# CVMI-Lab/DODA

Hardware: AMD Instinct MI355X
Metric: active-voxels/sec fwd+bwd SparseConv U-Net, ScanNet 2cm (higher is better)
Workload: dtype bf16; 1 GPU; cfgs/scannet SparseConv U-Net training step (voxel pooling + fwd + CE + bwd + SGD), 2 cm voxels, 4 scenes/GPU x ~150000 active voxels, random-init weights; global_batch=4, voxels_per_gpu=601279, points_per_gpu=781042, parallelism=dp1, n_classes=20, grad_sync=deferred multi-layer wgrad + bucketed all-reduce, collectives=none (single process), prefetch_gate=off, grad_exchange=no process group

## Files before the change

doda_amd/_lib.py:

```python
import ctypes as C
import os

_HERE = os.path.dirname(os.path.abspath(__file__))
LIB_PATH = os.path.join(_HERE, "libdoda_hip.so")

c_i32, c_i64, c_f32, c_sz, c_vp = C.c_int32, C.c_int64, C.c_float, C.c_size_t, C.c_void_p

_SIGNATURES = {
    "doda_abi_version": (c_i32, []),
    "doda_strerror": (C.c_char_p, [c_i32]),
    "doda_voxelize_idx_h": (c_i32, [c_vp, c_i32, c_i32, c_i32, c_i32, c_vp, C.POINTER(c_vp),
                                    C.POINTER(c_i32), C.POINTER(c_i32)]),
    "doda_voxelize_idx_fill_h": (c_i32, [c_vp, c_vp, c_vp, c_vp]),
    "doda_voxelize_idx_free_h": (None, [c_vp]),
    "doda_voxelize_idx_workspace_bytes": (c_sz, [c_i32]),
    "doda_voxelize_idx_assign": (c_i32, [c_vp, c_i32, c_i32, c_i32, c_vp, c_vp, c_vp, c_sz, c_vp]),
    "doda_voxelize_idx_fill": (c_i32, [c_vp, c_i32, c_i32, c_i32, c_i32, c_i32, c_vp, c_vp, c_vp,
                                       c_sz, c_vp]),
    "doda_voxelize_fp": (c_i32, [c_vp, c_vp, c_vp, c_i32, c_i32, c_i32, c_i32, c_vp]),
    "doda_voxelize_bp": (c_i32, [c_vp, c_vp, c_vp, c_i32, c_i32, c_i32, c_i32, c_vp]),
    "doda_voxelize_fp_rows": (c_i32, [c_vp, c_i32, c_vp, c_i32, c_vp, c_i32, c_i32, c_i32, c_vp, c_i32, c_i32, c_vp]),
    "doda_point_recover_fp": (c_i32, [c_vp, c_vp, c_vp, c_i32, c_i32, c_i32, c_vp]),
    "doda_point_recover_bp": (c_i32, [c_vp, c_vp, c_vp, c_i32, c_i32, c_i32, c_vp]),
    "doda_rulebook_workspace_bytes": (c_sz, [c_i32]),
# ... 121 lines not shown
    "doda_lovasz_bwd": (c_i32, [c_vp, c_i32, c_i32, c_i32, c_vp, c_vp, c_i32, c_vp, c_vp, c_vp, c_vp, c_vp, c_vp, c_vp, c_i32, c_vp]),
}
LOSS_SYMBOLS = tuple(LOSS_SIGNATURES)
LOSS_ABI_VERSION = 1
LOVASZ_MAX_CLASSES, LOVASZ_MAX_POINTS_PER_VOXEL = 32, 65535


class EvalScene(C.Structure):
    _fields_ = [("n_end", c_i32), ("m_end", c_i32), ("cell_base", c_i32), ("dims", c_i32 * 3), ("origin", c_f32 * 3),
                ("side", c_f32), ("inv_side", c_f32)]


EVAL_SIGNATURES = {
    "doda_eval_abi_version": (c_i32, []),
    "doda_eval_nn": (c_i32, [c_vp, c_vp, c_i64, c_vp, C.POINTER(EvalScene), c_i32, c_vp, c_vp, c_i64, c_vp, c_vp, c_vp]),
    "doda_eval_score_blocks": (c_i32, [c_i64]),
    "doda_eval_score": (c_i32, [c_vp, c_i32, c_i32, c_i32, c_vp, c_vp, c_i32, c_vp, c_i64, c_vp, c_vp, c_i64, c_i64, c_vp, c_vp, c_vp,
                                c_vp, c_i32, c_vp]),
}
EVAL_SYMBOLS = tuple(EVAL_SIGNATURES)
EVAL_ABI_VERSION = 1
EVAL_MAX_SCENES, EVAL_MAX_CELLS, EVAL_MAX_CLASSES = 32, 1 << 21, 32

c_u64p = C.POINTER(C.c_uint64)
SUBSAMPLE_SIGNATURES = {
    "doda_subsample_abi_version": (c_i32, []),
    "doda_subsample_workspace_bytes": (c_sz, [c_i64p, c_i32]),
    "doda_subsample_draw": (c_i32, [c_vp, c_vp, c_vp, c_vp, c_i64p, c_i32, c_i32p, c_u64p, C.c_uint32, c_vp, c_vp, c_vp, c_vp, c_vp,
                                    c_vp, c_sz, c_vp]),
}
SUBSAMPLE_SYMBOLS = tuple(SUBSAMPLE_SIGNATURES)
SUBSAMPLE_ABI_VERSION = 1
SUBSAMPLE_MAX_SEGMENTS, SUBSAMPLE_CHUNK = 64, 1024
OPT_TILE_KERNEL, OPT_WLDS_KERNEL, OPT_WDMA_KERNEL, OPT_TILE_PIPELINE, OPT_TILE_DUAL, OPT_CONV_UP = 1, 2, 3, 4, 5, 6
OPT_PRE_FWD_ROWS, OPT_PRE_BWD_ROWS = 7, 8
ABI_VERSION = 12

_ABIS = ((_SIGNATURES, "doda_abi_version", ABI_VERSION, "ABI"),
         (SELFTRAIN_SIGNATURES, "doda_st_abi_version", ST_ABI_VERSION, "self-training ABI"),
         (MIX_SIGNATURES, "doda_mix_abi_version", MIX_ABI_VERSION, "cuboid-mixing ABI"),
         (AUG_SIGNATURES, "doda_aug_abi_version", AUG_ABI_VERSION, "augmentation ABI"),
         (LOSS_SIGNATURES, "doda_loss_abi_version", LOSS_ABI_VERSION, "loss ABI"),
         (EVAL_SIGNATURES, "doda_eval_abi_version", EVAL_ABI_VERSION, "evaluation ABI"),
         (SUBSAMPLE_SIGNATURES, "doda_subsample_abi_version", SUBSAMPLE_ABI_VERSION, "subsample ABI"))

_lib = None


class DodaNativeError(RuntimeError):
    pass


def lib():
    global _lib
    if _lib is None:
        if not os.path.exists(LIB_PATH):
            raise DodaNativeError(
                "libdoda_hip.so is not built (%s). Run `python -m doda_amd.build` "
                "(hipcc, gfx950). doda_amd has no CPU fallback for its native ops." % LIB_PATH)
        handle = C.CDLL(LIB_PATH)
        for table, version_fn, version, what in _ABIS:
            for name, (res, args) in table.items():
                try:
                    fn = getattr(handle, name)
                except AttributeError as e:
                    raise DodaNativeError("libdoda_hip.so lacks symbol %s (stale build?)" % name) from e
                fn.restype = res
                fn.argtypes = args
            if getattr(handle, version_fn)() != version:
                raise DodaNativeError("libdoda_hip.so %s version mismatch" % what)
        _lib = handle
    return _lib


def check(status, what):
    if status != 0:
        msg = lib().doda_strerror(status).decode()
# ... 2 lines not shown
```

doda_amd/csrc/head.hip:

```cpp
#include "common.hpp"
#include "spconv_common.hpp"
#include "head_common.hpp"
#include "../../include/doda_selftrain.h"

namespace {

template <int ESZ, int C, int NK>
__global__ __launch_bounds__(HD_BLOCK, 4) void head_ce_fwd(const void *__restrict__ feats, int m, const float *__restrict__ weight,
                                                        const float *__restrict__ bias, int n_cls, const int32_t *__restrict__ v2p,
                                                        int v2p_ld, const long long *__restrict__ labels, long long ignore_index,
                                                        float *__restrict__ partial, int32_t *__restrict__ pred) {
    __shared__ float w[HD_MAX_K][HD_MAX_C], b[HD_MAX_K];
    __shared__ float red[2][HD_BLOCK / 64];
    hd_stage_weights<ESZ>(weight, bias, n_cls, C, w, b);
    float loss = 0.f, cnt = 0.f;
#pragma unroll 1
    for (long long v = (long long)blockIdx.x * HD_BLOCK + threadIdx.x; v < m; v += (long long)gridDim.x * HD_BLOCK) {
        asm volatile("" ::: "memory");
        float f[C], z[NK], mx;
        int arg;
        hd_load_row<ESZ, C>(feats, v, f);
        const int32_t *row = v2p + v * v2p_ld;
        const int np = row[0];
        hd_logits<C, NK>(w, b, n_cls, f, z, mx, arg);
        if (pred) pred[v] = arg;
        float s = 0.f;
#pragma unroll
        for (int k = 0; k < NK; ++k) s += __expf(z[k] - mx);
        const float lse = mx + __logf(s);
#pragma unroll 1
        for (int i = 0; i < np; ++i) {
            const long long lab = labels[row[1 + i]];
            if (lab != ignore_index && lab >= 0 && lab < n_cls) {
                float zy = 0.f;
#pragma unroll
                for (int k = 0; k < NK; ++k) zy = (int)lab == k ? z[k] : zy;
// ... 146 lines not shown
            }
            if (n_cls & 1) sdz[wid][n_cls - 1][lane] = r[n_cls - 1];
        } else {
#pragma unroll
            for (int c = 0; c < 16; ++c) sf[wid][c][lane] = 0;
            for (int k = 0; k < n_cls; ++k) sdz[wid][k][lane] = 0;
        }
        asm volatile("s_waitcnt lgkmcnt(0)" ::: "memory");
#pragma unroll
        for (int st = 0; st < 2; ++st) {
            const u32x4 bv = *reinterpret_cast<const u32x4 *>(&sf[wid][i][32 * st + 8 * g]);
#pragma unroll
            for (int t = 0; t < 2; ++t) {
                const u32x4 av = *reinterpret_cast<const u32x4 *>(&sdz[wid][16 * t + i][32 * st + 8 * g]);
                mma_bf16_k32(acc[t], av, bv);
            }
        }
        asm volatile("s_waitcnt lgkmcnt(0)" ::: "memory");
    }
    if (wid > 0) { red[wid - 1][0][lane] = acc[0]; red[wid - 1][1][lane] = acc[1]; }
    doda_sync();
    if (wid == 0) {
#pragma unroll
        for (int t = 0; t < 2; ++t) {
            f32x4 a = acc[t];
#pragma unroll
            for (int q = 0; q < 3; ++q) a += red[q][t][lane];
#pragma unroll
            for (int r = 0; r < 4; ++r) partial[(size_t)blockIdx.x * 512 + (size_t)(16 * t + 4 * g + r) * 16 + i] = a[r];
        }
    }
}

}

extern "C" int32_t doda_head_ce_blocks(int32_t m) { return hd_blocks(m > 0 ? m : 1); }

extern "C" int doda_head_ce_fwd(const void *feats, int32_t m, int32_t c, int32_t elem_bytes, const float *weight, const float *bias,
                                int32_t n_cls, const int32_t *v2p, int32_t v2p_ld, const int64_t *labels, int64_t ignore_index,
                                float *out, int32_t *pred, float *partial_ws, int32_t n_blocks, doda_stream_t stream) {
    if (!out) return DODA_ERR_INVALID;
    hipStream_t s = as_stream(stream);
    if (m == 0) { (void)hipMemsetAsync(out, 0, 8, s); return DODA_OK; }
    if (hd_args_bad(m, elem_bytes, v2p_ld, {feats, weight, v2p, labels, partial_ws}) || n_cls <= 0) return DODA_ERR_INVALID;
    if (c != 16 || n_cls > 32) return DODA_ERR_UNSUPPORTED;
    if (n_blocks != hd_blocks(m)) return DODA_ERR_WORKSPACE;
    HD_DISPATCH(head_ce_fwd, 16, n_blocks, feats, m, weight, bias, n_cls, v2p, v2p_ld, (const long long *)labels, (long long)ignore_index,
                partial_ws, pred);
    hipLaunchKernelGGL(head_ce_final, dim3(1), dim3(1024), 0, s, (const float *)partial_ws, n_blocks, out);
    return doda_check_launch();
}

extern "C" int doda_head_ce_bwd(const void *feats, int32_t m, int32_t c, int32_t elem_bytes, const float *weight, const float *bias,
                                int32_t n_cls, const int32_t *v2p, int32_t v2p_ld, const int64_t *labels, int64_t ignore_index,
                                const float *out, const float *grad, void *d_feats, void *dz, float *db_partial, int32_t n_blocks,
                                doda_stream_t stream) {
    if (m == 0) return DODA_OK;
    if (hd_args_bad(m, elem_bytes, v2p_ld, {feats, weight, v2p, labels, out, grad, d_feats, dz, db_partial}) || n_cls <= 0)
        return DODA_ERR_INVALID;
    if (c != 16 || n_cls > 32) return DODA_ERR_UNSUPPORTED;
    if (n_blocks != hd_blocks(m)) return DODA_ERR_WORKSPACE;
    hipStream_t s = as_stream(stream);
    HD_DISPATCH(head_ce_bwd, 16, n_blocks, feats, m, weight, bias, n_cls, v2p, v2p_ld, (const long long *)labels, (long long)ignore_index,
                out, grad, d_feats, dz, db_partial);
    return doda_check_launch();
}
// ... 29 lines not shown
```

doda_amd/csrc/spconv_gather.hip:

```cpp
#include <cstdio>
#include "common.hpp"
#include "tilebook.hpp"
#include "spconv_common.hpp"
#include "wgrad_backends.hpp"
#include <stdlib.h>

namespace {

struct F32 {
    typedef float elem;
    typedef f32x4 frag;
    static __device__ __forceinline__ frag zero() { return (frag){0.f, 0.f, 0.f, 0.f}; }
    static __device__ __forceinline__ elem from_float(float f) { return f; }
    static __device__ __forceinline__ float to_float(elem e) { return e; }
    static __device__ __forceinline__ void mma(f32x4 &acc, const frag &w, const frag &x) {
        mma_f32_k16<false>(acc, __builtin_bit_cast(u32x4, w), __builtin_bit_cast(u32x4, x));
    }
    static __device__ __forceinline__ void store4(elem *p, const f32x4 &v) {
        *reinterpret_cast<f32x4 *>(p) = v;
    }
};

struct BF16 {
    typedef unsigned short elem;
    typedef s16x4 frag;
    static __device__ __forceinline__ frag zero() { return (frag){0, 0, 0, 0}; }
    static __device__ __forceinline__ elem from_float(float f) { return f2bf(f); }
    static __device__ __forceinline__ float to_float(elem e) { return __uint_as_float((unsigned)e << 16); }
    static __device__ __forceinline__ void mma(f32x4 &acc, const frag &w, const frag &x) {
        acc = __builtin_amdgcn_mfma_f32_16x16x16bf16_1k(w, x, acc, 0, 0, 0);
    }
    static __device__ __forceinline__ void store4(elem *p, const f32x4 &v) {
        s16x4 o;
#pragma unroll
        for (int q = 0; q < 4; ++q) o[q] = (short)f2bf(v[q]);
        *reinterpret_cast<s16x4 *>(p) = o;
    }
// ... 92 lines not shown
            else f = d.w[((long long)((d.layout & 3) == 2 ? d.K - 1 - o : o) * d.nc + col) * d.kc + c];
        }
        v[q] = T::from_float(f);
    }
    reinterpret_cast<typename T::frag *>(d.out)[e] = v;
}

__global__ __launch_bounds__(256) void pack_weights_multi(const PackDesc *__restrict__ descs,
                                                          const int *__restrict__ blk_end, int n_desc) {
    int lo = 0, hi = n_desc - 1;
    while (lo < hi) {
        const int mid = (lo + hi) >> 1;
        if ((int)blockIdx.x < blk_end[mid]) hi = mid; else lo = mid + 1;
    }
    const PackDesc d = descs[lo];
    const int first = lo == 0 ? 0 : blk_end[lo - 1];
    const unsigned e = (unsigned)(blockIdx.x - first) * 256u + threadIdx.x;
    if (d.layout & 0x20) {
        if (e >= (unsigned)d.K * (unsigned)d.NB * 32u) return;
        const unsigned r = e >> 5, o = r / (unsigned)d.NB;
        reinterpret_cast<u32x4_t *>(d.out)[e] =
            pack_wide_frag(d.w, d.K, d.kc, d.nc, d.layout & 3, (int)o, 0, (int)(r - o * (unsigned)d.NB), (int)(e & 31));
        return;
    }
    const unsigned total = (unsigned)d.K * (unsigned)d.n_chunk * (unsigned)d.NB * 64u;
    if (e >= total) return;
    if (d.layout & 0x10) {
        const unsigned r = e >> 6, r1 = r / (unsigned)d.NB, nb = r - r1 * (unsigned)d.NB;
        const unsigned o = r1 / (unsigned)d.n_chunk, cc = r1 - o * (unsigned)d.n_chunk;
        reinterpret_cast<u32x4_t *>(d.out)[e] =
            pack_wide_frag(d.w, d.K, d.kc, d.nc, d.layout & 3, (int)o, (int)cc, (int)nb, (int)(e & 63));
    } else if (d.elem_bytes == 4) pack_one<F32>(d, e);
    else pack_one<BF16>(d, e);
}

constexpr int MAX_K = 27;

template <class T, int NBW, int S>
__global__ __launch_bounds__(256) void conv_gather(const typename T::elem *__restrict__ x, int kc,
                                                   const typename T::frag *__restrict__ wp, int nc,
                                                   int NB, const int32_t *__restrict__ tbl, int ld,
                                                   int K, int n_out,
                                                   typename T::elem *__restrict__ y, int vec_ok,
                                                   const typename T::elem *__restrict__ res) {
    typedef typename T::frag frag;
    typedef typename T::elem elem;
    constexpr int TM = 4 * 16 * S;
    __shared__ int32_t idx_tile[MAX_K * TM];

    const int lane = threadIdx.x & 63, wid = threadIdx.x >> 6;
    const int i = lane & 15, g = lane >> 4;
    const int n_nbg = (NB + NBW - 1) / NBW;
    const int item = xcd_work_item(blockIdx.x, gridDim.x);
    const long long r0 = (long long)(item / n_nbg) * TM;
    const int nb0 = (item % n_nbg) * NBW;

    for (int e = threadIdx.x; e < K * TM; e += 256) {
        const int o = e / TM, r = e - o * TM;
        idx_tile[e] = (r0 + r < n_out) ? tbl[(long long)o * ld + r0 + r] : -1;
    }
    doda_sync();

    const int wrow = wid * 16 * S;
    if (r0 + wrow >= n_out) return;

    unsigned int active = 0;
// ... 716 lines not shown
}

extern "C" size_t doda_spconv_pack_desc_bytes(void) { return sizeof(PackDesc); }

extern "C" int doda_spconv_pack_plan_h(void *descs_h, int32_t n_desc, int32_t *blk_end_h,
                                       int32_t *total_blocks) {
    if (!descs_h || !blk_end_h || !total_blocks || n_desc <= 0) return DODA_ERR_INVALID;
    PackDesc *d = (PackDesc *)descs_h;
    long long acc = 0;
    for (int k = 0; k < n_desc; ++k) {
        if (d[k].K <= 0 || d[k].K > MAX_K || d[k].kc <= 0 || d[k].nc <= 0 || (d[k].layout & ~3) ||
            (d[k].layout & 3) > 2 || (d[k].elem_bytes != 2 && d[k].elem_bytes != 4))
            return DODA_ERR_INVALID;
        const PackGeometry g = pack_geometry(d[k].K, d[k].kc, d[k].nc, d[k].elem_bytes);
        d[k].layout |= g.mode;
        d[k].n_chunk = g.n_chunk;
        d[k].NB = g.NB;
        acc += div_up(g.frags, 256);
        if (acc > 0x7fffffff) return DODA_ERR_UNSUPPORTED;
        blk_end_h[k] = (int32_t)acc;
    }
    *total_blocks = (int32_t)acc;
    return DODA_OK;
}

extern "C" int doda_spconv_pack_multi(const void *descs_dev, const int32_t *blk_end_dev,
                                      int32_t n_desc, int32_t total_blocks, doda_stream_t stream) {
    if (!descs_dev || !blk_end_dev || n_desc <= 0 || total_blocks <= 0) return DODA_ERR_INVALID;
    hipLaunchKernelGGL(pack_weights_multi, dim3(total_blocks), dim3(256), 0, as_stream(stream),
                       (const PackDesc *)descs_dev, blk_end_dev, n_desc);
    return doda_check_launch();
}

static bool *gather_switch(int32_t option) {
    switch (option) {
    case DODA_OPT_TILE_KERNEL: return &gather_switches().tile;
    case DODA_OPT_WLDS_KERNEL: return &gather_switches().wlds;
    case DODA_OPT_TILE_PIPELINE: return &gather_switches().tile_pipeline;
    case DODA_OPT_TILE_DUAL: return &gather_switches().tile_dual;
    case DODA_OPT_CONV_UP: return &gather_switches().conv_up;
    default: return nullptr;
    }
}
extern "C" int doda_set_option(int32_t option, int32_t value) {
    if (bool *sw = gather_switch(option)) { *sw = value != 0; return DODA_OK; }
    switch (option) {
    case DODA_OPT_WDMA_KERNEL: doda_wdma::set_enabled(value != 0); return DODA_OK;
    case DODA_OPT_PRE_FWD_ROWS: doda_layers::set_fwd_rows(value); return DODA_OK;
    case DODA_OPT_PRE_BWD_ROWS: doda_layers::set_bwd_rows(value); return DODA_OK;
    default: return DODA_ERR_INVALID;
    }
}
extern "C" int32_t doda_get_option(int32_t option) {
    if (const bool *sw = gather_switch(option)) return *sw ? 1 : 0;
    switch (option) {
    case DODA_OPT_WDMA_KERNEL: return doda_wdma::enabled() ? 1 : 0;
    case DODA_OPT_PRE_FWD_ROWS: return (int32_t)doda_layers::fwd_rows();
    case DODA_OPT_PRE_BWD_ROWS: return (int32_t)doda_layers::bwd_rows();
    default: return -1;
    }
}

extern "C" size_t doda_spconv_stats_capacity(int32_t n_out) { return n_out > 0 ? (size_t)div_up(n_out, 16) : 1; }

namespace doda_gather {
const GatherSwitches &switches() { return gather_switches(); }
// ... 60 lines not shown
```

doda_amd/csrc/spconv_wdma.hip:

```cpp
#include "tilebook.hpp"
#include "spconv_common.hpp"
#include "wgrad_common.hpp"
#include <stdlib.h>
#include <type_traits>
#include <string.h>

namespace {

constexpr int WD_WAVES = 16;
constexpr int WD_ROWS_BYTES = (TB_UMAX + 1) * 32;
constexpr int WD_LIDX_BYTES = TB_LIDX_BYTES;
constexpr int WD_DY_BYTES = TB_T * 32;
constexpr int WD_UNITS_BYTES = 2 * TB_K * 256 * 4;
constexpr int WD_BUF_BYTES = (WD_ROWS_BYTES + WD_LIDX_BYTES + WD_DY_BYTES) > WD_UNITS_BYTES ? (WD_ROWS_BYTES + WD_LIDX_BYTES + WD_DY_BYTES)
                                                                                           : WD_UNITS_BYTES;
static_assert(WD_LIDX_BYTES % 1024 == 0, "whole DMA pieces");
constexpr int WD_UNITS = 2 * TB_K;
constexpr int WD_MAX_UNITS = (WD_UNITS + WD_WAVES - 1) / WD_WAVES;
constexpr int WD_MAX_JOBS = 16;
static_assert(WD_BUF_BYTES % 16 == 0 && 2 * WD_BUF_BYTES + 64 <= 160 * 1024, "two tile buffers per CU");
static_assert(WD_UNITS * 256 * 4 <= WD_BUF_BYTES, "the final exchange re-uses ONE tile buffer (the other may be a DMA target)");

struct WdJob { const void *x, *dy; float *part; unsigned x_stride, dy_stride; int first_rank, pad; };
struct WdJobs { int n; WdJob j[WD_MAX_JOBS]; };
// ... 232 lines not shown
            const int o = e >> 8, c = e & 255;
            dst[e] = ex[(2 * o) * 256 + c] + ex[(2 * o + 1) * 256 + c];
        }
        asm volatile("s_waitcnt lgkmcnt(0)\n\ts_barrier" ::: "memory");
        if (tid < 2) reinterpret_cast<u32x4 *>(smem + bufsel * WD_BUF_BYTES)[tid] = (u32x4){0u, 0u, 0u, 0u};
        asm volatile("s_waitcnt lgkmcnt(0)\n\ts_barrier" ::: "memory");
    };

    bool nl_cur = __builtin_amdgcn_readfirstlane((int)la[0]) == -2;
    for (int item = 0; item < n_items; item += 2) {
        asm volatile("s_waitcnt vmcnt(0)" : "+v"(lb) : : "memory");
        asm volatile("s_waitcnt lgkmcnt(0)\n\ts_barrier" ::: "memory");
        {
            const bool nl_next = __builtin_amdgcn_readfirstlane((int)lb[0]) == -2;
            body(item, nl_cur, lb, la);
            nl_cur = nl_next;
        }
        if (item + 1 == n_items || (start + item + 1) % nt == 0) flush((start + item) / nt, item & 1, start + item);
        if (item + 1 >= n_items) break;
        asm volatile("s_waitcnt vmcnt(0)" : "+v"(la) : : "memory");
        asm volatile("s_waitcnt lgkmcnt(0)\n\ts_barrier" ::: "memory");
        {
            const bool nl_next = __builtin_amdgcn_readfirstlane((int)la[0]) == -2;
            body(item + 1, nl_cur, la, lb);
            nl_cur = nl_next;
        }
        if (item + 2 == n_items || (start + item + 2) % nt == 0) flush((start + item + 1) / nt, (item + 1) & 1, start + item + 1);
    }
    asm volatile("s_waitcnt vmcnt(0)" ::: "memory");
}

struct WdRJob { const float *part; float *dw; int accumulate, ldo, ldc, n_part; };
struct WdRJobs { WdRJob j[WD_MAX_JOBS]; };

__global__ __launch_bounds__(512) void wgrad_dma_reduce(const WdRJobs jobs) {
    __shared__ float red[16][32];
    const WdRJob d = jobs.j[blockIdx.y];
    const int n_part = d.n_part;
    const int jx = threadIdx.x & 31, p = threadIdx.x >> 5;
    const int e = blockIdx.x * 32 + jx;
    float a[8];
#pragma unroll
    for (int q = 0; q < 8; ++q) a[q] = 0.f;
    int b = p;
    for (; b + 7 * 16 < n_part; b += 8 * 16) {
#pragma unroll
        for (int q = 0; q < 8; ++q) a[q] += d.part[(size_t)(b + q * 16) * (TB_K * 256) + e];
    }
    for (int q = 0; b < n_part; b += 16, ++q) a[q & 7] += d.part[(size_t)b * (TB_K * 256) + e];
    red[p][jx] = ((a[0] + a[1]) + (a[2] + a[3])) + ((a[4] + a[5]) + (a[6] + a[7]));
    doda_sync();
    if (p == 0) {
        float v = 0.f;
#pragma unroll
        for (int q = 0; q < 16; ++q) v += red[q][jx];
        float *dst = d.dw + (size_t)(e >> 8) * d.ldo + (size_t)((e >> 4) & 15) * d.ldc + (e & 15);
        *dst = d.accumulate ? *dst + v : v;
    }
}

static_assert(WP_TILE_ROWS == TB_T && WP_TILE_K == TB_K, "wgrad_plan.hpp restates these constants");

struct Block { const void *x, *dy; float *dw; int x_stride, dy_stride, ldo, ldc, accumulate; };
struct WdArgs { WdJobs jobs; WdRJobs red; };

}

namespace doda_wdma {
// ... 38 lines not shown
            const int nj = l.n_blocks - first < WD_MAX_JOBS ? l.n_blocks - first : WD_MAX_JOBS;
            WdArgs a;
            ::memset(&a, 0, sizeof(a));
            a.jobs.n = nj;
            int first_rank[WD_MAX_JOBS], count[WD_MAX_JOBS];
            for (int k = 0; k < nj; ++k) { first_rank[k] = -1; count[k] = 0; }
            const long long N = (long long)nj * nt;
            if (N >= groups) {
                for (int r = 0; r < groups; ++r) {
                    const long long st = (long long)r * N / groups, en = (long long)(r + 1) * N / groups;
                    for (long long b = st / nt; b <= (en - 1) / nt; ++b) {
                        if (first_rank[b] < 0) first_rank[b] = r;
                        ++count[b];
                    }
                }
            } else {
                for (int k = 0; k < nj; ++k) { first_rank[k] = 0; count[k] = nt; }
            }
            for (int k = 0; k < nj; ++k) {
                const Block &b = blocks[first + k];
                float *pp = (float *)(part + used);
                used += (size_t)count[k] * TB_K * 256 * sizeof(float);
                a.jobs.j[k] = WdJob{b.x, b.dy, pp, (unsigned)b.x_stride, (unsigned)b.dy_stride, first_rank[k], 0};
                a.red.j[k] = WdRJob{pp, b.dw, b.accumulate, b.ldo, b.ldc, count[k]};
            }
            const unsigned char *bytes = (const unsigned char *)&a;
            p.args.insert(p.args.end(), bytes, bytes + sizeof(a));
        }
    }
}

int launch(const Plan &p, const doda_wgrad_job *jobs, hipStream_t s) {
    const WdArgs *a = (const WdArgs *)p.args.data();
    for (const Plan::Launch &l : p.launches) {
        const doda_wgrad_job &j0 = jobs[p.order[l.first_job]];
        const TileBookView tb = tilebook_view(const_cast<void *>(j0.tilebook), j0.n_rows);
        for (int first = 0; first < l.n_blocks; first += WD_MAX_JOBS, ++a) {
            doda_wgrad::trace("wgrad_dma16", wdma_groups(j0.n_rows), 1024, a->jobs.n);
            hipLaunchKernelGGL(wgrad_dma16, dim3(wdma_groups(j0.n_rows)), dim3(1024), 0, s, a->jobs, j0.tbl, j0.ld, j0.n_rows, tb);
            doda_wgrad::trace("wgrad_dma_reduce", TB_K * 256 / 32 * a->jobs.n, 512, a->jobs.n);
            hipLaunchKernelGGL(wgrad_dma_reduce, dim3(TB_K * 256 / 32, a->jobs.n), dim3(512), 0, s, a->red);
        }
    }
    return doda_check_launch();
}

}
```

doda_amd/model.py:

```python
import functools
from collections import OrderedDict
from types import SimpleNamespace

import torch
from torch import nn
from torch.autograd import Function

from torch.nn.modules import module as _torch_module

from . import ops as _ops
from . import pointgroup_ops, spconv
from .spconv import conv as _cv
from .spconv import functional as Fsp
from .spconv.modules import SparseModule


def default_cfg(n_classes=20, in_channel=3, mid_channel=16, block_reps=2, block_residual=True,
                use_xyz=False, voxel_mode=4):
    backbone = SimpleNamespace(in_channel=in_channel, mid_channel=mid_channel, block_reps=block_reps,
                               block_residual=block_residual, use_xyz=use_xyz)
    return SimpleNamespace(MODEL=SimpleNamespace(BACKBONE=backbone),
                           COMMON_CLASSES=SimpleNamespace(n_classes=n_classes),
                           DATA_CONFIG=SimpleNamespace(
                               DATA_PROCESSOR=SimpleNamespace(voxel_mode=voxel_mode),
# ... 472 lines not shown
            d_b = d_scores.sum(0)
        return d_feats, d_w, d_b, None, None


class _FusedCE(Function):
    @staticmethod
    def forward(ctx, scores, labels, ignore_index):
        scores = scores.contiguous()
        out, lse = _ops.cross_entropy_fwd(scores, labels, ignore_index)
        ctx.save_for_backward(scores, labels, lse, out)
        ctx.ignore_index = ignore_index
        return out[0]

    @staticmethod
    def backward(ctx, grad):
        scores, labels, lse, out = ctx.saved_tensors
        g = grad.reshape(1).to(torch.float32).contiguous()
        return _ops.cross_entropy_bwd(scores, labels, lse, out, g, ctx.ignore_index), None, None


class _VoxelHeadCE(Function):

    @staticmethod
    def forward(ctx, feats, weight, bias, v2p, labels, ignore_index):
        out, pred = _ops.head_ce_fwd(feats, weight, bias, v2p, labels, ignore_index)
        ctx.save_for_backward(feats, weight, bias, v2p, labels, out)
        ctx.ignore_index = ignore_index
        ctx.mark_non_differentiable(pred)
        return out[0], pred

    @staticmethod
    def backward(ctx, grad, _grad_pred):
        feats, weight, bias, v2p, labels, out = ctx.saved_tensors
        d_feats, dz, d_b = _ops.head_ce_bwd(feats, weight, bias, v2p, labels, ctx.ignore_index, out, grad.reshape(1).to(torch.float32))
        return _ops.head_grads(ctx.needs_input_grad, feats, weight, bias, d_feats, dz, None, d_b)


FUSED_HEAD_LOSS = _os.environ.get("DODA_FUSED_HEAD_LOSS", "1") == "1"


def cross_entropy(scores, labels, ignore_index=255):
    if (scores.is_cuda and scores.dtype == torch.float32 and scores.dim() == 2 and scores.shape[1] <= 64
            and labels.dtype == torch.int64 and scores.shape[0] > 0):
        return _FusedCE.apply(scores, labels.contiguous(), int(ignore_index))
    valid = labels != ignore_index
    logp = torch.log_softmax(scores.float(), dim=1)
    picked = logp.gather(1, labels.clamp(0, scores.shape[1] - 1).unsqueeze(1)).squeeze(1)
    return -(picked * valid).sum() / valid.sum().clamp(min=1)


LOSS_KINDS = ("cross_entropy", "lovasz")


def loss_kind_of(cfg):
    opt = getattr(cfg, "OPTIMIZATION", None)
    kind = "cross_entropy" if opt is None else (opt.get("loss", "cross_entropy") if hasattr(opt, "get")
                                                else getattr(opt, "loss", "cross_entropy"))
    if kind not in LOSS_KINDS:
        raise NotImplementedError("OPTIMIZATION.loss: %r (cross_entropy | lovasz)" % (kind,))
    return kind


def criterion_of(model):
    net = model.module if hasattr(model, "module") else model
    return getattr(net, "criterion", cross_entropy)


# ... 283 lines not shown
```

doda_amd/ops.py:

```python
import ctypes as C
import os

import numpy as np
import torch

from ._lib import LOVASZ_MAX_POINTS_PER_VOXEL, DodaNativeError, check, lib


_raw_stream = getattr(torch._C, "_cuda_getCurrentRawStream", None)


def _stream():
    if _raw_stream is not None:
        return _raw_stream(torch.cuda.current_device())
    return torch.cuda.current_stream().cuda_stream


def _p(t):
    return t.data_ptr() if t is not None else None


def _need_cuda(*ts):
    for t in ts:
        if not t.is_cuda:
            raise RuntimeError("doda_amd native ops need device (ROCm) tensors; got a %s tensor — "
                               "there is no CPU fallback" % t.device)


_WS = {}


def _ws(nbytes, device):
    nbytes = max(int(nbytes), 256)
    key = (device, _stream())
    buf = _WS.get(key)
    if buf is None or buf.numel() < nbytes:
        buf = torch.empty(max(nbytes, 1 << 20), dtype=torch.uint8, device=device)
        _WS[key] = buf
    return buf
# ... 342 lines not shown

def bn_fwd_final(stats, m, eps, momentum, running_mean=None, running_var=None, num_batches_tracked=None):
    _need_cuda(stats)
    rows, _, c = stats.shape
    mean = torch.empty(c, dtype=torch.float32, device=stats.device)
    invstd = torch.empty(c, dtype=torch.float32, device=stats.device)
    check(lib().doda_bn_fwd_final(_p(stats), rows, int(m), c, float(eps), float(momentum),
                                  _p(running_mean) if running_mean is not None else None,
                                  _p(running_var) if running_var is not None else None,
                                  _p(num_batches_tracked) if num_batches_tracked is not None else None,
                                  _p(mean), _p(invstd), _stream()), "doda_bn_fwd_final")
    return mean, invstd


class PackPlan:

    def __init__(self, entries, device):
        import numpy as np
        l = lib()
        n = len(entries)
        dsz = l.doda_spconv_pack_desc_bytes()
        assert dsz == 48
        desc = np.zeros(n, dtype=np.dtype([("w", "<u8"), ("out", "<u8"), ("K", "<i4"), ("kc", "<i4"),
                                           ("nc", "<i4"), ("layout", "<i4"), ("esz", "<i4"),
                                           ("n_chunk", "<i4"), ("NB", "<i4"), ("pad", "<i4")]))
        self.outputs = []
        for k, (w, K, kc, nc, layout, esz) in enumerate(entries):
            if not (w.is_cuda and w.dtype == torch.float32 and w.is_contiguous() and w.numel() == K * kc * nc):
                raise RuntimeError("PackPlan: weights must be contiguous fp32 device tensors")
            out = torch.empty(l.doda_spconv_gather_workspace_bytes(K, kc, nc, esz), dtype=torch.uint8,
                              device=device)
            self.outputs.append(out)
            desc[k] = (w.data_ptr(), out.data_ptr(), K, kc, nc, layout, esz, 0, 0, 0)
        blk_end = np.zeros(n, dtype=np.int32)
        total = C.c_int32()
        check(l.doda_spconv_pack_plan_h(desc.ctypes.data, n, blk_end.ctypes.data, C.byref(total)),
              "doda_spconv_pack_plan_h")
        self.n, self.total = n, int(total.value)
        self.desc_dev = torch.from_numpy(desc.view(np.uint8).copy()).to(device)
        self.blk_dev = torch.from_numpy(blk_end).to(device)

    def run(self):
        check(lib().doda_spconv_pack_multi(_p(self.desc_dev), _p(self.blk_dev), self.n, self.total,
                                           _stream()), "doda_spconv_pack_multi")


class _WgradJob(C.Structure):
    _fields_ = [("a", C.c_void_p), ("b", C.c_void_p), ("tbl", C.c_void_p), ("dw", C.c_void_p),
                ("ca", C.c_int32), ("cb", C.c_int32), ("ld", C.c_int32), ("K", C.c_int32),
                ("n_rows", C.c_int32), ("elem_bytes", C.c_int32),
                ("pair_in", C.c_void_p), ("pair_out", C.c_void_p), ("pair_num", C.c_void_p),
                ("pair_ld", C.c_int32), ("n_a", C.c_int32), ("flags", C.c_int32), ("reserved", C.c_int32),
                ("pair_seg", C.c_void_p), ("pair_seg_nt", C.c_int32), ("reserved2", C.c_int32),
                ("tilebook", C.c_void_p)]


WGRAD_ACCUMULATE = 1


class WgradPlan:

    def __init__(self, jobs):
        self.outputs = spconv_wgrad_multi(jobs, _plan=self)

    def run(self):
        check(lib().doda_spconv_wgrad_multi(C.addressof(self._arr), self._n, _p(self._ws), self._ws.numel(), _p(self._desc),
                                            self._desc.numel(), _stream()), "doda_spconv_wgrad_multi")
        return self.outputs


def spconv_wgrad_multi(jobs, _plan=None):
    if not jobs:
        return []
    arr = (_WgradJob * len(jobs))()
    outs, keep = [], []
# ... 256 lines not shown
def cross_entropy_fwd(logits, labels, ignore_index):
    _need_cuda(logits)
    _need_cuda(labels)
    if logits.dtype != torch.float32 or labels.dtype != torch.int64 or logits.dim() != 2:
        raise RuntimeError("cross_entropy: logits float32 [N,C], labels int64 [N]")
    logits, labels = logits.contiguous(), labels.contiguous()
    n, c = logits.shape
    lse = torch.empty(n, dtype=torch.float32, device=logits.device)
    out = torch.empty(2, dtype=torch.float32, device=logits.device)
    ws = _ws(lib().doda_cross_entropy_workspace_bytes(n), logits.device)
    check(lib().doda_cross_entropy_fwd(_p(logits), _p(labels), n, c, int(ignore_index), _p(lse), _p(out), _p(ws),
                                       ws.numel(), _stream()), "doda_cross_entropy_fwd")
    return out, lse


def cross_entropy_bwd(logits, labels, lse, out, grad, ignore_index):
    n, c = logits.shape
    d = torch.empty_like(logits)
    check(lib().doda_cross_entropy_bwd(_p(logits), _p(labels), _p(lse), _p(out), _p(grad), n, c, int(ignore_index),
                                       _p(d), _stream()), "doda_cross_entropy_bwd")
    return d


def _head_args(what, feats, weight, bias, v2p=None, labels=None):
    _feat_ok(feats, "feats")
    lists = v2p is not None
    _need_cuda(weight, *((v2p, labels) if lists else ()))
    if weight.dtype != torch.float32 or (lists and (v2p.dtype != torch.int32 or labels.dtype != torch.int64 or v2p.dim() != 2)):
        raise RuntimeError("%s: weight float32 [n_cls, c]%s" % (what, ", v2p int32 [m, 1 + max_active], labels int64 [points]" if lists else ""))
    cont = lambda t: t.contiguous() if t is not None else None
    return feats.contiguous(), weight.contiguous(), cont(bias), cont(v2p), cont(labels)


def _head_bwd(blocks, feats, weight, bias, want_lo, launch):
    feats, weight = feats.contiguous(), weight.contiguous()
    (m, c), n_cls = feats.shape, weight.shape[0]
    nb = int(blocks(m))
    d_feats = torch.empty_like(feats)
    dz = torch.empty((m, n_cls), dtype=feats.dtype, device=feats.device)
    dz_lo = torch.empty_like(dz) if want_lo else None
    dbp = torch.empty((nb, n_cls), dtype=torch.float32, device=feats.device)
    launch((_p(feats), m, c, feats.element_size(), _p(weight), _p(bias.contiguous() if bias is not None else None), n_cls),
           d_feats, dz, dz_lo, dbp, nb)
    return d_feats, dz, dz_lo, dbp.sum(0)


def head_ce_fwd(feats, weight, bias, v2p, labels, ignore_index, want_pred=True):
    feats, weight, bias, v2p, labels = _head_args("head_ce", feats, weight, bias, v2p, labels)
    m, c = feats.shape
    nb = int(lib().doda_head_ce_blocks(m))
    out = torch.empty(2, dtype=torch.float32, device=feats.device)
    pred = torch.empty(m, dtype=torch.int32, device=feats.device) if want_pred else None
    ws = torch.empty(2 * nb, dtype=torch.float32, device=feats.device)
    check(lib().doda_head_ce_fwd(_p(feats), m, c, feats.element_size(), _p(weight), _p(bias), weight.shape[0], _p(v2p), v2p.shape[1],
                                 _p(labels), int(ignore_index), _p(out), _p(pred), _p(ws), nb, _stream()), "doda_head_ce_fwd")
    return out, pred


def head_ce_bwd(feats, weight, bias, v2p, labels, ignore_index, out, grad):
    v2p, labels = v2p.contiguous(), labels.contiguous()
    d_feats, dz, _, d_b = _head_bwd(lib().doda_head_ce_blocks, feats, weight, bias, False, lambda head, d_feats, dz, dz_lo, dbp, nb: check(
        lib().doda_head_ce_bwd(*head, _p(v2p), v2p.shape[1], _p(labels), int(ignore_index), _p(out), _p(grad.contiguous()), _p(d_feats),
                               _p(dz), _p(dbp), nb, _stream()), "doda_head_ce_bwd"))
    return d_feats, dz, d_b


def head_dw(feats, dz):
    m, c = feats.shape
    n_cls = dz.shape[1]
    if feats.dtype == torch.bfloat16 and c == 16 and n_cls <= 32:
        nb = int(lib().doda_head_dw_blocks(m))
        part = torch.empty((nb, 32, 16), dtype=torch.float32, device=feats.device)
        check(lib().doda_head_dw_bf16(_p(feats.contiguous()), _p(dz.contiguous()), m, c, n_cls, _p(part), nb, _stream()), "doda_head_dw_bf16")
        return part.sum(0)[:n_cls]
    ident = torch.arange(m, dtype=torch.int32, device=feats.device).view(1, m)
    return spconv_wgrad(feats.contiguous(), dz, ident, m)[0].t()


def head_grads(needs, feats, weight, bias, d_feats, dz, dz_lo, d_b):
    d_w = None
    if needs[1]:
        d_w = head_dw(feats, dz)
        if dz_lo is not None:
            d_w = d_w + head_dw(feats, dz_lo)
        d_w = d_w.to(weight.dtype)
    return (d_feats if needs[0] else None), d_w, (d_b if bias is not None and needs[2] else None), None, None, None


def lovasz_fwd(feats, weight, bias, v2p, labels, ignore_index, want_grad=True):
    feats, weight, bias, v2p, labels = _head_args("lovasz", feats, weight, bias, v2p, labels)
    m, c = feats.shape
    n_cls = weight.shape[0]
    out = torch.empty(2, dtype=torch.float32, device=feats.device)
    pred = torch.empty(m, dtype=torch.int32, device=feats.device)
    gitem = torch.empty((m, n_cls, 2), dtype=torch.float32, device=feats.device) if want_grad else None
    nbytes = int(lib().doda_lovasz_workspace_bytes(m, n_cls))
    if nbytes == 0:
        raise DodaNativeError("doda_lovasz_fwd: %d voxels x %d classes is outside the compiled range" % (m, n_cls))
    ws = _ws(nbytes, feats.device)
    check(lib().doda_lovasz_fwd(_p(feats), m, c, feats.element_size(), _p(weight), _p(bias), n_cls, _p(v2p), v2p.shape[1], _p(labels),
                                int(ignore_index), _p(out), _p(pred), _p(gitem), _p(ws), ws.numel(), _stream()), "doda_lovasz_fwd")
    return out, pred, gitem


def lovasz_bwd(feats, weight, bias, gitem, out, grad):
    return _head_bwd(lib().doda_lovasz_blocks, feats, weight, bias, feats.dtype == torch.bfloat16, lambda head, d_feats, dz, dz_lo, dbp, nb: check(
        lib().doda_lovasz_bwd(*head, _p(gitem), _p(out), _p(grad.contiguous()), _p(d_feats), _p(dz), _p(dz_lo), _p(dbp), nb, _stream()),
        "doda_lovasz_bwd"))


def voxel_confidence(feats, weight, bias):
    feats, weight, bias, _, _ = _head_args("voxel_confidence", feats, weight, bias)
    if weight.dim() != 2 or weight.shape[1] != feats.shape[1]:
# ... 328 lines not shown
```

Baseline: 138.3 million voxels/s.

## Fuse head grad reductions, pair weight packing, batch wgrad reduce launches

Adds a single kernel that reduces both the bias and weight-gradient partials of the CE head, replacing two separate torch sum reductions. Weight packing now uses one kernel pass per weight that emits both the forward and the transposed backward packed layouts from an LDS-staged tile, so the fp32 weights are read once instead of twice. The wgrad DMA reduce launches are deferred and batched into up to 112 jobs per launch, which cuts launch count at the cost of a larger kernel-argument struct. The aim is to remove small-kernel launch overhead and redundant weight reads in the training step.

```diff
diff --git a/doda_amd/_lib.py b/doda_amd/_lib.py
--- a/doda_amd/_lib.py
+++ b/doda_amd/_lib.py
@@ -177,6 +177,17 @@
 SUBSAMPLE_SYMBOLS = tuple(SUBSAMPLE_SIGNATURES)
 SUBSAMPLE_ABI_VERSION = 1
 SUBSAMPLE_MAX_SEGMENTS, SUBSAMPLE_CHUNK = 64, 1024
+
+STEP_SIGNATURES = {
+    "doda_step_abi_version": (c_i32, []),
+    "doda_step_head_bwd_final": (c_i32, [c_vp, c_i32, c_vp, c_i32, c_i32, c_i32, c_vp, c_vp, c_vp]),
+    "doda_step_pack_desc_bytes": (c_sz, []),
+    "doda_step_pack_plan_h": (c_i32, [c_vp, c_i32, C.POINTER(c_i32), C.POINTER(c_i32)]),
+    "doda_step_pack_multi": (c_i32, [c_vp, c_i32, c_i32, c_i32, c_vp]),
+}
+STEP_SYMBOLS = tuple(STEP_SIGNATURES)
+STEP_ABI_VERSION = 1
+STEP_PACK_MAX_COLS = 256
 OPT_TILE_KERNEL, OPT_WLDS_KERNEL, OPT_WDMA_KERNEL, OPT_TILE_PIPELINE, OPT_TILE_DUAL, OPT_CONV_UP = 1, 2, 3, 4, 5, 6
 OPT_PRE_FWD_ROWS, OPT_PRE_BWD_ROWS = 7, 8
 ABI_VERSION = 12
@@ -187,7 +198,8 @@
          (AUG_SIGNATURES, "doda_aug_abi_version", AUG_ABI_VERSION, "augmentation ABI"),
          (LOSS_SIGNATURES, "doda_loss_abi_version", LOSS_ABI_VERSION, "loss ABI"),
          (EVAL_SIGNATURES, "doda_eval_abi_version", EVAL_ABI_VERSION, "evaluation ABI"),
-         (SUBSAMPLE_SIGNATURES, "doda_subsample_abi_version", SUBSAMPLE_ABI_VERSION, "subsample ABI"))
+         (SUBSAMPLE_SIGNATURES, "doda_subsample_abi_version", SUBSAMPLE_ABI_VERSION, "subsample ABI"),
+         (STEP_SIGNATURES, "doda_step_abi_version", STEP_ABI_VERSION, "step ABI"))
 
 _lib = None
 
diff --git a/doda_amd/csrc/head.hip b/doda_amd/csrc/head.hip
--- a/doda_amd/csrc/head.hip
+++ b/doda_amd/csrc/head.hip
@@ -2,6 +2,7 @@
 #include "spconv_common.hpp"
 #include "head_common.hpp"
 #include "../../include/doda_selftrain.h"
+#include "../../include/doda_step.h"
 
 namespace {
 
@@ -214,6 +215,39 @@
     }
 }
 
+__global__ __launch_bounds__(1024) void head_bwd_final(const float *__restrict__ db_partial, int n_db, const float *__restrict__ dw_partial,
+                                                       int n_dw, int n_cls, int c, float *__restrict__ db, float *__restrict__ dw) {
+    __shared__ double red[1024];
+    const bool bias = (int)blockIdx.x == n_cls;
+    const int width = bias ? n_cls : c, rows = bias ? n_db : n_dw;
+    const size_t stride = bias ? (size_t)n_cls : (size_t)32 * c;
+    const float *src = bias ? db_partial : dw_partial + (size_t)blockIdx.x * c;
+    float *dst = bias ? db : dw + (size_t)blockIdx.x * c;
+    const int RG = 1024 / width;
+    const int rg = threadIdx.x / width, j = threadIdx.x - rg * width;
+    double a = 0.0;
+    if (rg < RG)
+#pragma unroll 8
+        for (int r = rg; r < rows; r += RG) a += (double)src[(size_t)r * stride + j];
+    red[threadIdx.x] = a;
+    doda_sync();
+    if ((int)threadIdx.x < width) {
+        double v = 0.0;
+        for (int q = 0; q < RG; ++q) v += red[q * width + threadIdx.x];
+        dst[threadIdx.x] = (float)v;
+    }
+}
+
+}
+
+extern "C" int32_t doda_step_abi_version(void) { return DODA_STEP_ABI_VERSION; }
+
+extern "C" int doda_step_head_bwd_final(const float *db_partial, int32_t n_db, const float *dw_partial, int32_t n_dw, int32_t n_cls, int32_t c,
+                                   float *db, float *dw, doda_stream_t stream) {
+    if (!db_partial || !dw_partial || !db || !dw || n_db <= 0 || n_dw <= 0 || n_cls <= 0 || c <= 0) return DODA_ERR_INVALID;
+    if (n_cls > 32 || c > 32) return DODA_ERR_UNSUPPORTED;
+    hipLaunchKernelGGL(head_bwd_final, dim3(n_cls + 1), dim3(1024), 0, as_stream(stream), db_partial, n_db, dw_partial, n_dw, n_cls, c, db, dw);
+    return doda_check_launch();
 }
 
 extern "C" int32_t doda_head_ce_blocks(int32_t m) { return hd_blocks(m > 0 ? m : 1); }
diff --git a/doda_amd/csrc/spconv_gather.hip b/doda_amd/csrc/spconv_gather.hip
--- a/doda_amd/csrc/spconv_gather.hip
+++ b/doda_amd/csrc/spconv_gather.hip
@@ -3,6 +3,7 @@
 #include "tilebook.hpp"
 #include "spconv_common.hpp"
 #include "wgrad_backends.hpp"
+#include "../../include/doda_step.h"
 #include <stdlib.h>
 
 namespace {
@@ -161,6 +162,95 @@
             pack_wide_frag(d.w, d.K, d.kc, d.nc, d.layout & 3, (int)o, (int)cc, (int)nb, (int)(e & 63));
     } else if (d.elem_bytes == 4) pack_one<F32>(d, e);
     else pack_one<BF16>(d, e);
+}
+
+constexpr int PP_ROWS = 32, PP_MAX_COLS = DODA_STEP_PACK_MAX_COLS;
+struct PackPairDesc {
+    const float *w;
+    void *out_f, *out_b;
+    int K, a, b, bwd_layout, elem_bytes;
+    int mode_f, n_chunk_f, NB_f, mode_b, n_chunk_b, NB_b, blk_end;
+};
+
+template <bool TR>
+__device__ __forceinline__ void pp_emit(const float *s, int LD, int r0, int a, int b, int mode, int esz, int n_chunk, int NB,
+                                        int o_out, int cc0, int cc1, int nb0, int nb1, void *out) {
+    auto get = [&](int c, int col) -> float {
+        if (TR) return (col < a && c < b) ? s[(col - r0) * LD + c] : 0.f;
+        return (c < a && col < b) ? s[(c - r0) * LD + col] : 0.f;
+    };
+    const int L = mode == 0x20 ? 32 : 64;
+    const unsigned nnb = (unsigned)(nb1 - nb0), total = (unsigned)(cc1 - cc0) * nnb * (unsigned)L;
+    for (unsigned t = threadIdx.x; t < total; t += 256) {
+        const int lane = (int)(t & (unsigned)(L - 1));
+        const unsigned u = t / (unsigned)L, ccl = u / nnb;
+        const int nb = nb0 + (int)(u - ccl * nnb), cc = cc0 + (int)ccl;
+        const int i = lane & 15, g = lane >> 4, col = nb * 16 + i;
+        if (mode != 0) {
+            unsigned short h[8];
+#pragma unroll
+            for (int q = 0; q < 8; ++q) h[q] = f2bf(get(cc * 32 + 8 * g + q, col));
+            u32x4_t r;
+#pragma unroll
+            for (int q = 0; q < 4; ++q) r[q] = (unsigned)h[2 * q] | ((unsigned)h[2 * q + 1] << 16);
+            const size_t e = mode == 0x20 ? ((size_t)o_out * NB + nb) * 32 + lane : (((size_t)o_out * n_chunk + cc) * NB + nb) * 64 + lane;
+            reinterpret_cast<u32x4_t *>(out)[e] = r;
+        } else {
+            float f[4];
+#pragma unroll
+            for (int q = 0; q < 4; ++q) f[q] = get(cc * 16 + 4 * g + q, col);
+            const size_t e = (((size_t)o_out * n_chunk + cc) * NB + nb) * 64 + lane;
+            if (esz == 4) reinterpret_cast<F32::frag *>(out)[e] = (F32::frag){f[0], f[1], f[2], f[3]};
+            else {
+                BF16::frag v;
+#pragma unroll
+                for (int q = 0; q < 4; ++q) v[q] = (short)f2bf(f[q]);
+                reinterpret_cast<BF16::frag *>(out)[e] = v;
+            }
+        }
+    }
+}
+
+__global__ __launch_bounds__(256) void pack_weights_pair(const PackPairDesc *__restrict__ descs, int n_desc, int max_cols) {
+    extern __shared__ float s[];
+    int lo = 0, hi = n_desc - 1;
+    while (lo < hi) {
+        const int mid = (lo + hi) >> 1;
+        if ((int)blockIdx.x < descs[mid].blk_end) hi = mid; else lo = mid + 1;
+    }
+    const PackPairDesc d = descs[lo];
+    if (d.b > max_cols) return;
+    const unsigned unit = blockIdx.x - (lo == 0 ? 0 : descs[lo - 1].blk_end);
+    const unsigned nrc = (unsigned)(d.a + PP_ROWS - 1) / PP_ROWS;
+    const int o = (int)(unit / nrc), rc = (int)(unit - (unsigned)o * nrc), r0 = rc * PP_ROWS;
+    const int nr = d.a - r0 < PP_ROWS ? d.a - r0 : PP_ROWS;
+    const int LD = d.b + 1;
+    const float *src = d.w + ((size_t)o * d.a + r0) * d.b;
+    const unsigned n = (unsigned)nr * (unsigned)d.b;
+    if ((d.b & 3) == 0 && ((uintptr_t)d.w & 15) == 0) {
+        for (unsigned q = threadIdx.x; q < n / 4; q += 256) {
+            const f32x4 v = reinterpret_cast<const f32x4 *>(src)[q];
+            const unsigned r = (q * 4) / (unsigned)d.b, c = q * 4 - r * (unsigned)d.b;
+            float *p = s + r * LD + c;
+            p[0] = v[0]; p[1] = v[1]; p[2] = v[2]; p[3] = v[3];
+        }
+    } else {
+        for (unsigned k = threadIdx.x; k < n; k += 256) {
+            const unsigned r = k / (unsigned)d.b;
+            s[r * LD + (k - r * (unsigned)d.b)] = src[k];
+        }
+    }
+    doda_sync();
+    if (d.out_f) {
+        const int per = d.mode_f == 0 ? 2 : 1;
+        const int cc0 = rc * per, cc1 = cc0 + per < d.n_chunk_f ? cc0 + per : d.n_chunk_f;
+        if (cc0 < cc1) pp_emit<false>(s, LD, r0, d.a, d.b, d.mode_f, d.elem_bytes, d.n_chunk_f, d.NB_f, o, cc0, cc1, 0, d.NB_f, d.out_f);
+    }
+    if (d.out_b) {
+        const int nb0 = rc * 2, nb1 = nb0 + 2 < d.NB_b ? nb0 + 2 : d.NB_b;
+        pp_emit<true>(s, LD, r0, d.a, d.b, d.mode_b, d.elem_bytes, d.n_chunk_b, d.NB_b, d.bwd_layout == 2 ? d.K - 1 - o : o, 0,
+                      d.n_chunk_b, nb0, nb1, d.out_b);
+    }
 }
 
 constexpr int MAX_K = 27;
@@ -943,6 +1033,40 @@
     return doda_check_launch();
 }
 
+extern "C" size_t doda_step_pack_desc_bytes(void) { return sizeof(PackPairDesc); }
+
+extern "C" int doda_step_pack_plan_h(void *descs_h, int32_t n_desc, int32_t *total_blocks, int32_t *max_cols) {
+    if (!descs_h || !total_blocks || !max_cols || n_desc <= 0) return DODA_ERR_INVALID;
+    PackPairDesc *d = (PackPairDesc *)descs_h;
+    long long acc = 0;
+    int widest = 0;
+    for (int k = 0; k < n_desc; ++k) {
+        if (!d[k].w || (!d[k].out_f && !d[k].out_b) || d[k].K <= 0 || d[k].K > MAX_K || d[k].a <= 0 || d[k].b <= 0 ||
+            (d[k].out_b && d[k].bwd_layout != 1 && d[k].bwd_layout != 2) || (d[k].elem_bytes != 2 && d[k].elem_bytes != 4))
+            return DODA_ERR_INVALID;
+        if (d[k].b > PP_MAX_COLS) return DODA_ERR_UNSUPPORTED;
+        const PackGeometry f = pack_geometry(d[k].K, d[k].a, d[k].b, d[k].elem_bytes), b = pack_geometry(d[k].K, d[k].b, d[k].a, d[k].elem_bytes);
+        d[k].mode_f = f.mode; d[k].n_chunk_f = f.n_chunk; d[k].NB_f = f.NB;
+        d[k].mode_b = b.mode; d[k].n_chunk_b = b.n_chunk; d[k].NB_b = b.NB;
+        acc += (long long)d[k].K * div_up(d[k].a, PP_ROWS);
+        if (acc > 0x7fffffff) return DODA_ERR_UNSUPPORTED;
+        d[k].blk_end = (int)acc;
+        if (d[k].b > widest) widest = d[k].b;
+    }
+    *total_blocks = (int32_t)acc;
+    *max_cols = widest;
+    return DODA_OK;
+}
+
+extern "C" int doda_step_pack_multi(const void *descs_dev, int32_t n_desc, int32_t total_blocks, int32_t max_cols, doda_stream_t stream) {
+    if (!descs_dev || n_desc <= 0 || total_blocks <= 0 || max_cols <= 0) return DODA_ERR_INVALID;
+    if (max_cols > PP_MAX_COLS) return DODA_ERR_UNSUPPORTED;
+    const size_t lds = (size_t)PP_ROWS * (max_cols + 1) * sizeof(float);
+    hipLaunchKernelGGL(pack_weights_pair, dim3(total_blocks), dim3(256), lds, as_stream(stream), (const PackPairDesc *)descs_dev, n_desc,
+                       max_cols);
+    return doda_check_launch();
+}
+
 static bool *gather_switch(int32_t option) {
     switch (option) {
     case DODA_OPT_TILE_KERNEL: return &gather_switches().tile;
diff --git a/doda_amd/csrc/spconv_wdma.hip b/doda_amd/csrc/spconv_wdma.hip
--- a/doda_amd/csrc/spconv_wdma.hip
+++ b/doda_amd/csrc/spconv_wdma.hip
@@ -288,8 +288,11 @@
 
 struct WdRJob { const float *part; float *dw; int accumulate, ldo, ldc, n_part; };
 struct WdRJobs { WdRJob j[WD_MAX_JOBS]; };
-
-__global__ __launch_bounds__(512) void wgrad_dma_reduce(const WdRJobs jobs) {
+constexpr int WD_RED_MAX_JOBS = 112;
+struct WdRAll { WdRJob j[WD_RED_MAX_JOBS]; };
+static_assert(sizeof(WdRAll) <= 3584, "kernel arguments: 4 KB with room for the hidden ones");
+
+__global__ __launch_bounds__(512) void wgrad_dma_reduce(const WdRAll jobs) {
     __shared__ float red[16][32];
     const WdRJob d = jobs.j[blockIdx.y];
     const int n_part = d.n_part;
@@ -394,16 +397,30 @@
 
 int launch(const Plan &p, const doda_wgrad_job *jobs, hipStream_t s) {
     const WdArgs *a = (const WdArgs *)p.args.data();
+    const WdArgs *const a0 = a;
     for (const Plan::Launch &l : p.launches) {
         const doda_wgrad_job &j0 = jobs[p.order[l.first_job]];
         const TileBookView tb = tilebook_view(const_cast<void *>(j0.tilebook), j0.n_rows);
         for (int first = 0; first < l.n_blocks; first += WD_MAX_JOBS, ++a) {
             doda_wgrad::trace("wgrad_dma16", wdma_groups(j0.n_rows), 1024, a->jobs.n);
             hipLaunchKernelGGL(wgrad_dma16, dim3(wdma_groups(j0.n_rows)), dim3(1024), 0, s, a->jobs, j0.tbl, j0.ld, j0.n_rows, tb);
-            doda_wgrad::trace("wgrad_dma_reduce", TB_K * 256 / 32 * a->jobs.n, 512, a->jobs.n);
-            hipLaunchKernelGGL(wgrad_dma_reduce, dim3(TB_K * 256 / 32, a->jobs.n), dim3(512), 0, s, a->red);
-        }
-    }
+        }
+    }
+    WdRAll red;
+    ::memset(&red, 0, sizeof(red));
+    int n = 0;
+    auto flush = [&]() {
+        if (n == 0) return;
+        doda_wgrad::trace("wgrad_dma_reduce", TB_K * 256 / 32 * n, 512, n);
+        hipLaunchKernelGGL(wgrad_dma_reduce, dim3(TB_K * 256 / 32, n), dim3(512), 0, s, red);
+        n = 0;
+    };
+    for (const WdArgs *q = a0; q != a; ++q)
+        for (int k = 0; k < q->jobs.n; ++k) {
+            red.j[n++] = q->red.j[k];
+            if (n == WD_RED_MAX_JOBS) flush();
+        }
+    flush();
     return doda_check_launch();
 }
 
diff --git a/doda_amd/model.py b/doda_amd/model.py
--- a/doda_amd/model.py
+++ b/doda_amd/model.py
@@ -528,7 +528,8 @@
     @staticmethod
     def backward(ctx, grad, _grad_pred):
         feats, weight, bias, v2p, labels, out = ctx.saved_tensors
-        d_feats, dz, d_b = _ops.head_ce_bwd(feats, weight, bias, v2p, labels, ctx.ignore_index, out, grad.reshape(1).to(torch.float32))
+        d_feats, dz, d_b = _ops.head_ce_bwd(feats, weight, bias, v2p, labels, ctx.ignore_index, out, grad.reshape(1).to(torch.float32),
+                                            db_rows=True)
         return _ops.head_grads(ctx.needs_input_grad, feats, weight, bias, d_feats, dz, None, d_b)
 
 
diff --git a/doda_amd/ops.py b/doda_amd/ops.py
--- a/doda_amd/ops.py
+++ b/doda_amd/ops.py
@@ -4,7 +4,7 @@
 import numpy as np
 import torch
 
-from ._lib import LOVASZ_MAX_POINTS_PER_VOXEL, DodaNativeError, check, lib
+from ._lib import LOVASZ_MAX_POINTS_PER_VOXEL, STEP_PACK_MAX_COLS, DodaNativeError, check, lib
 
 
 _raw_stream = getattr(torch._C, "_cuda_getCurrentRawStream", None)
@@ -413,6 +413,29 @@
                               device=device)
             self.outputs.append(out)
             desc[k] = (w.data_ptr(), out.data_ptr(), K, kc, nc, layout, esz, 0, 0, 0)
+        stored = [(kc, nc) if layout == 0 else (nc, kc) for (_, _, kc, nc, layout, _) in entries]
+        self.paired = all(0 < b <= STEP_PACK_MAX_COLS for _, b in stored) and all(e[4] in (0, 1, 2) for e in entries)
+        if self.paired:
+            assert l.doda_step_pack_desc_bytes() == 72
+            slots = {}
+            rows = []
+            for k, ((w, K, kc, nc, layout, esz), (a, b)) in enumerate(zip(entries, stored)):
+                key, side = (w.data_ptr(), K, a, b, esz), 0 if layout == 0 else 1
+                row = slots.get(key)
+                if row is None or row[side] is not None:
+                    row = slots[key] = [None, None]
+                    rows.append((key, row))
+                row[side] = k
+            pd = np.zeros(len(rows), dtype=np.dtype([("w", "<u8"), ("out_f", "<u8"), ("out_b", "<u8"), ("K", "<i4"), ("a", "<i4"),
+                                                     ("b", "<i4"), ("bwd_layout", "<i4"), ("esz", "<i4"), ("plan", "<i4", (7,))]))
+            for r, ((wp, K, a, b, esz), (kf, kb)) in enumerate(rows):
+                pd[r] = (wp, self.outputs[kf].data_ptr() if kf is not None else 0, self.outputs[kb].data_ptr() if kb is not None else 0,
+                         K, a, b, entries[kb][4] if kb is not None else 0, esz, (0,) * 7)
+            total, cols = C.c_int32(), C.c_int32()
+            check(l.doda_step_pack_plan_h(pd.ctypes.data, len(rows), C.byref(total), C.byref(cols)), "doda_step_pack_plan_h")
+            self.n, self.total, self.max_cols = len(rows), int(total.value), int(cols.value)
+            self.desc_dev = torch.from_numpy(pd.view(np.uint8).copy()).to(device)
+            return
         blk_end = np.zeros(n, dtype=np.int32)
         total = C.c_int32()
         check(l.doda_spconv_pack_plan_h(desc.ctypes.data, n, blk_end.ctypes.data, C.byref(total)),
@@ -422,6 +445,9 @@
         self.blk_dev = torch.from_numpy(blk_end).to(device)
 
     def run(self):
+        if self.paired:
+            check(lib().doda_step_pack_multi(_p(self.desc_dev), self.n, self.total, self.max_cols, _stream()), "doda_step_pack_multi")
+            return
         check(lib().doda_spconv_pack_multi(_p(self.desc_dev), _p(self.blk_dev), self.n, self.total,
                                            _stream()), "doda_spconv_pack_multi")
 
@@ -744,7 +770,7 @@
     return feats.contiguous(), weight.contiguous(), cont(bias), cont(v2p), cont(labels)
 
 
-def _head_bwd(blocks, feats, weight, bias, want_lo, launch):
+def _head_bwd(blocks, feats, weight, bias, want_lo, launch, db_rows=False):
     feats, weight = feats.contiguous(), weight.contiguous()
     (m, c), n_cls = feats.shape, weight.shape[0]
     nb = int(blocks(m))
@@ -754,7 +780,7 @@
     dbp = torch.empty((nb, n_cls), dtype=torch.float32, device=feats.device)
     launch((_p(feats), m, c, feats.element_size(), _p(weight), _p(bias.contiguous() if bias is not None else None), n_cls),
            d_feats, dz, dz_lo, dbp, nb)
-    return d_feats, dz, dz_lo, dbp.sum(0)
+    return d_feats, dz, dz_lo, (dbp if db_rows else dbp.sum(0))
 
 
 def head_ce_fwd(feats, weight, bias, v2p, labels, ignore_index, want_pred=True):
@@ -769,28 +795,55 @@
     return out, pred
 
 
-def head_ce_bwd(feats, weight, bias, v2p, labels, ignore_index, out, grad):
+def head_ce_bwd(feats, weight, bias, v2p, labels, ignore_index, out, grad, db_rows=False):
     v2p, labels = v2p.contiguous(), labels.contiguous()
     d_feats, dz, _, d_b = _head_bwd(lib().doda_head_ce_blocks, feats, weight, bias, False, lambda head, d_feats, dz, dz_lo, dbp, nb: check(
         lib().doda_head_ce_bwd(*head, _p(v2p), v2p.shape[1], _p(labels), int(ignore_index), _p(out), _p(grad.contiguous()), _p(d_feats),
-                               _p(dz), _p(dbp), nb, _stream()), "doda_head_ce_bwd"))
+                               _p(dz), _p(dbp), nb, _stream()), "doda_head_ce_bwd"), db_rows)
     return d_feats, dz, d_b
+
+
+def _head_dw_mfma(feats, dz):
+    return feats.dtype == torch.bfloat16 and feats.shape[1] == 16 and dz.shape[1] <= 32
+
+
+def head_dw_partials(feats, dz):
+    (m, c), n_cls = feats.shape, dz.shape[1]
+    nb = int(lib().doda_head_dw_blocks(m))
+    part = torch.empty((nb, 32, 16), dtype=torch.float32, device=feats.device)
+    check(lib().doda_head_dw_bf16(_p(feats.contiguous()), _p(dz.contiguous()), m, c, n_cls, _p(part), nb, _stream()), "doda_head_dw_bf16")
+    return part
+
+
+def head_bwd_final(db_rows, dw_part, n_cls):
+    _need_cuda(db_rows, dw_part)
+    db_rows, dw_part = db_rows.contiguous(), dw_part.contiguous()
+    c = dw_part.shape[2]
+    if db_rows.dtype != torch.float32 or dw_part.dtype != torch.float32 or db_rows.shape[1] != n_cls or dw_part.shape[1] != 32:
+        raise RuntimeError("head_bwd_final: float32 db_rows [blocks, n_cls] and dw_part [blocks, 32, c]")
+    d_b = torch.empty(n_cls, dtype=torch.float32, device=db_rows.device)
+    d_w = torch.empty((n_cls, c), dtype=torch.float32, device=db_rows.device)
+    check(lib().doda_step_head_bwd_final(_p(db_rows), db_rows.shape[0], _p(dw_part), dw_part.shape[0], n_cls, c, _p(d_b), _p(d_w),
+                                         _stream()), "doda_step_head_bwd_final")
+    return d_b, d_w
 
 
 def head_dw(feats, dz):
     m, c = feats.shape
     n_cls = dz.shape[1]
-    if feats.dtype == torch.bfloat16 and c == 16 and n_cls <= 32:
-        nb = int(lib().doda_head_dw_blocks(m))
-        part = torch.empty((nb, 32, 16), dtype=torch.float32, device=feats.device)
-        check(lib().doda_head_dw_bf16(_p(feats.contiguous()), _p(dz.contiguous()), m, c, n_cls, _p(part), nb, _stream()), "doda_head_dw_bf16")
-        return part.sum(0)[:n_cls]
+    if _head_dw_mfma(feats, dz):
+        return head_dw_partials(feats, dz).sum(0)[:n_cls]
     ident = torch.arange(m, dtype=torch.int32, device=feats.device).view(1, m)
     return spconv_wgrad(feats.contiguous(), dz, ident, m)[0].t()
 
 
 def head_grads(needs, feats, weight, bias, d_feats, dz, dz_lo, d_b):
     d_w = None
+    if d_b is not None and d_b.dim() == 2:
+        if needs[1] and dz_lo is None and feats.shape[0] > 0 and _head_dw_mfma(feats, dz):
+            d_b, d_w = head_bwd_final(d_b, head_dw_partials(feats, dz), dz.shape[1])
+            return (d_feats if needs[0] else None), d_w.to(weight.dtype), (d_b if bias is not None and needs[2] else None), None, None, None
+        d_b = d_b.sum(0)
     if needs[1]:
         d_w = head_dw(feats, dz)
         if dz_lo is not None:
diff --git a/include/doda_step.h b/include/doda_step.h
--- /dev/null
+++ b/include/doda_step.h
@@ -0,0 +1,29 @@
+#ifndef DODA_STEP_H
+#define DODA_STEP_H
+
+#include <stddef.h>
+#include <stdint.h>
+
+#include "doda_hip.h"
+
+#ifdef __cplusplus
+extern "C" {
+#endif
+
+#define DODA_STEP_ABI_VERSION 1
+
+int32_t doda_step_abi_version(void);
+
+int doda_step_head_bwd_final(const float *db_partial, int32_t n_db, const float *dw_partial, int32_t n_dw, int32_t n_cls, int32_t c,
+                             float *db, float *dw, doda_stream_t stream);
+
+#define DODA_STEP_PACK_MAX_COLS 256
+size_t doda_step_pack_desc_bytes(void);
+int doda_step_pack_plan_h(void *descs_h, int32_t n_desc, int32_t *total_blocks, int32_t *max_cols);
+int doda_step_pack_multi(const void *descs_dev, int32_t n_desc, int32_t total_blocks, int32_t max_cols, doda_stream_t stream);
+
+#ifdef __cplusplus
+}
+#endif
+
+#endif
```

New measurement: 138.0 million voxels/s. About the same (-0.2%).
